# OpenResearchInstitute/ka9q-sdr

Measured on AMD Instinct MI355X. Metric: input Msamples/s + channels @ real-time, 16384-pt overlap-save, higher is better.
Workload: dtype f32

## Files before the change

ka9q_sdr_amd/csrc/kq_bank.cpp:

```cpp
#include <cstdarg>

#include "kq_bank.hpp"

using namespace kq::bank;

namespace {
thread_local std::string g_err;

int ilog2(unsigned v) {
  int l = 0;
  while ((1u << l) < v) l++;
  return l;
}
}

void kq_internal_set_error(const char *fmt, ...) {
  char buf[512];
  va_list ap;
  va_start(ap, fmt);
  vsnprintf(buf, sizeof buf, fmt, ap);
  va_end(ap);
  g_err = buf;
}

// ... 255 lines not shown
    if (b->alloc(&b->pl2[k].filt, C * B * g.olen, true)) return -1;
    if (b->alloc(&b->pl2[k].n0raw, C * B, true)) return -1;
    if (b->alloc(&b->pl2[k].if_power, B * (1 + kq::kEnergySplitMax), true)) return -1;
    if (g.pl_n > 0 && b->alloc(&b->pl2[k].plout, C * B * g.pl_l, true)) return -1;
  }
  b->pl = b->pl2[0];
  if (b->alloc(&b->energy_state, 2, true)) return -1;
  if (kq::full16k_paired_supported(g) && b->alloc(&b->win_paired, (size_t)(g.M - 1) + (size_t)B * g.L, true)) return -1;
  for (int *&l : b->list_dev)
    if (b->alloc(&l, C, true)) return -1;
  for (kq_bank::CtlQueue &q : b->ctl)
    for (int k = 0; k < kq_bank::CtlQueue::kDepth; k++)
      if (b->alloc_pinned(&q.buf[k], kq_bank::CtlQueue::kBytes) || b->new_event(&q.applied[k], hipEventDisableTiming)) return -1;
  {
    kq_bank::DesignQueue &d = b->dq;
    size_t const per_job = (size_t)g.Ndec * sizeof(float2);
    d.max_jobs = (unsigned)std::max<size_t>(1, std::min<size_t>(kq_bank::DesignQueue::kMax, ((size_t)64 << 20) / per_job));
    if (b->alloc(&d.scratch, (size_t)d.max_jobs * g.Ndec, true)) return -1;
    if (b->alloc(&d.ng_next, 2 * C, true)) return -1;
    for (int k = 0; k < kq_bank::DesignQueue::kDepth; k++)
      if (b->alloc_pinned(&d.pin[k], kq_bank::DesignQueue::kMax * (sizeof(kq::DesignJob) + sizeof(kq::DesignTarget))) ||
          b->new_event(&d.read[k], hipEventDisableTiming))
        return -1;
    for (hipEvent_t &e : d.ng_moved)
      if (b->new_event(&e, hipEventDisableTiming)) return -1;
    if (g.Ndec <= 16384 && kq::design_prepare(g.olen, g.Mdec)) return -1;
  }
  if (b->alloc(&b->list_active_dev, C, true)) return -1;
  if (b->alloc(&b->list_active_ds_dev, C, true)) return -1;
  if (b->alloc(&b->chd.fflags, C, true)) return -1;
  if (b->alloc(&b->list_unswept_dev, C, true)) return -1;
  if (b->alloc(&b->list_swept_dev, C, true)) return -1;
  if (b->fwd_mode == KQ_FWD_PRUNED && b->alloc(&b->chan_tw, C * kq::pruned_table_elems(g), true)) return -1;
  KQ_TRY(hipStreamSynchronize(b->stream));
  if (g.pl_n > 0) {
    int const PL_M = g.pl_n - g.pl_l + 1;
    std::vector<kq::cfloat> r(g.pl_n / 2 + 1, kq::cfloat(0, 0));
    for (int j = 0; j <= g.pl_n / 2; j++) {
      float const f = (float)j * g.dsamprate / g.Ndec;
      if (f > 0 && f < 300) r[j] = 1;
    }
    if (kq::window_rfilter(g.pl_l, PL_M, r, 2.0)) return -1;
    KQ_TRY(hipMemcpy(b->chd.plresp, r.data(), r.size() * sizeof(float2), hipMemcpyHostToDevice));
  }
  {
    std::vector<float> nanv(C, NAN);
    KQ_TRY(hipMemcpy(b->chd.plfreq, nanv.data(), C * sizeof(float), hipMemcpyHostToDevice));
  }
  return 0;
}
}

kq_bank *kq_bank_create(const kq_bank_config *cfg) {
  if (create_check(cfg)) return nullptr;
  kq::DeviceScope dev_scope_(cfg->device);
  {
    int cur = -1;
    if (hipGetDevice(&cur) != hipSuccess || cur != cfg->device) {
      kq_internal_set_error("hipSetDevice(%d) failed", cfg->device);
      return nullptr;
    }
  }
  kq_bank *b = new kq_bank();
  b->cfg = *cfg;
  b->chans.reserve(cfg->max_channels);
  if (create_geometry(b) || create_alloc(b)) {
// ... 79 lines not shown
```

ka9q_sdr_amd/csrc/kq_bank.hpp:

```cpp
#pragma once
#include <hip/hip_runtime.h>

#include <chrono>
#include <cmath>
#include <cstdio>
#include <cstdlib>
#include <cstring>
#include <map>
#include <mutex>
#include <string>
#include <unordered_map>
#include <vector>

#include "kq_design.hpp"
#include "kq_device.hpp"
#include "kq_host.hpp"

#define LAUNCH_CHECK(what)                                                                        \
  do {                                                                                            \
    hipError_t e_ = hipGetLastError();                                                            \
    if (e_ != hipSuccess) {                                                                       \
      kq_internal_set_error("kernel launch failed in %s: %s", what, hipGetErrorString(e_));       \
      return -1;                                                                                  \
    }                                                                                             \
// ... 55 lines not shown
  int histx_dev[kq::kOldLevels] = {-1, -1, -1, -1};
  static_assert(kq::kOldLevels == 4, "histx_dev's initialiser");
  bool active = true;
  kq_out_rtp_state out_rtp{};
  int out_type;
  std::vector<kq::cfloat> resp, aresp;
  float noise_gain;
  int pll_slot = -1;
  int n0slot = -1;
  int lk = -1, lpos = -1, apos = -1;
  bool patched = false;
  double r_eff = 0;
};

struct EventPair {
  hipEvent_t a, b;
};

}

struct kq_bank : kq::HostSide {
  std::recursive_mutex mu;
  kq_bank_config cfg;
  kq::Geom g;
  int fwd_mode = KQ_FWD_FULL;
  uint64_t calls = 0;
  int64_t n_abs = 0;
  int64_t out_abs = 0;
  unsigned last_blocks = 0;

  const float2 *tw = nullptr;
  float2 *chan_tw = nullptr;
  bool chan_tw_dirty = true;
  kq::ChanDev chd{};
  kq::Planes pl{};
  float *energy_state = nullptr;
  float2 *win_paired = nullptr;
  bool use64k = false;
  kq::Big64 big{};
  float *fmout = nullptr;
  float *fm_hist[2] = {nullptr, nullptr};
  int fm_hist_cur = 0;

  int timing = 0;
  kq_host_timing host_acc = {};
  const char *worst_holder = "";
  std::vector<kq::bank::EventPair> ev_filter, ev_demod, ev_ingest;
  size_t ev_used[3] = {0, 0, 0};
  kq_timing acc = {};

  struct CtlQueue {
    static constexpr size_t kBytes = 1u << 20, kMaxRec = 4096;
    static constexpr int kDepth = 4;
    unsigned char *buf[kDepth] = {};
    hipEvent_t applied[kDepth] = {};
    bool applied_set[kDepth] = {};
    int cur = 0;
    unsigned nrec = 0;
    size_t used = 0;
    std::unordered_map<unsigned long long, unsigned> at;
  };
  CtlQueue ctl[2];
  struct DesignQueue {
    static constexpr unsigned kMax = 1024;
    static constexpr int kDepth = 4;
    unsigned char *pin[kDepth] = {};
// ... 228 lines not shown
```

ka9q_sdr_amd/csrc/kq_bank_call.cpp:

```cpp
#include "kq_bank.hpp"

using namespace kq::bank;

namespace kq::bank {

void harvest_slot(kq_bank *b, int slot) {
  if (!b->stage_timed[slot]) return;
  b->stage_timed[slot] = false;
  float ms = 0;
  if (hipEventElapsedTime(&ms, b->stage_t0[slot], b->stage_ev[slot]) == hipSuccess && ms > 0) {
    b->acc.filter_ms += ms;
    if (ms > b->acc.filter_max_ms) {
      b->acc.filter_max_ms = ms;
      b->acc.filter_max_submit_ms = b->stage_submit_ms[slot];
      b->acc.filter_max_launch = b->stage_launch[slot];
    }
  } else
    (void)hipGetLastError();
}

void note_retune(kq_bank *b, int ch) {
  HostChan &h = b->chans[ch];
  int64_t const hist = (int64_t)b->g.M - 1;
  if (h.retuned && h.hist_old == hist) return;
// ... 327 lines not shown
    for (int c = 0; c < k.C; c++) {
      if (!b->chans[c].active) continue;
      bool const isb = b->chans[c].cfg.demod_type == KQ_LINEAR_DEMOD && b->chans[c].cfg.isb;
      for (unsigned i = 0; i < k.nblocks; i++) {
        const float2 *X = k.spectrum + (size_t)i * g.N;
        size_t const cb = (size_t)c * g.max_blocks + i;
        if (b->cfg.compute_n0)
          kq::launch_n0_single(b->stream, X, g.N, g.samprate, b->chans[c].cfg.low, b->chans[c].cfg.high, k.pl.n0raw + cb);
        kq::launch_slave_bank(b->stream, X, k.chd.resp + (size_t)c * g.Ndec, k.pl.filt + cb * g.olen, g.N, g.Ndec, g.olen, isb ? 2 : 1,
                              b->tw, g.tw_log2);
      }
    }
  } else if (b->fwd_mode == KQ_FWD_PRUNED) {
    if (b->chan_tw_dirty) {
      kq::launch_pruned_tables(b->stream, g, k.chd, b->chan_tw, k.C);
      b->chan_tw_dirty = false;
    }
    if (kq::pruned_carries_iir(g)) iir_arm(b, k);
    kq::launch_filter_pruned(b->stream, g, k.chd, k.pl, k.window, b->chan_tw, act.n, nblocks, k.swept_pruned, act.list, b->big.iir);
    b->big.iir = kq::IirArgs{};
    if (k.nret > 0) {
      if (g.N > 16384)
        kq::launch_filter_split(b->stream, g, k.chd, k.pl, k.window, b->tw, k.nret, (int)k.nredo, k.retune_list);
      else
        full_launch(b, k, k.nret, (int)k.nredo, k.retune_list, 0, false);
    }
  } else if (b->use64k) {
    launch64k(b, k, act.n, nblocks, act.list, k.plain);
    if (k.plain && k.nret > 0) launch64k(b, k, k.nret, (int)k.nredo, k.retune_list, false);
  } else if (g.N > 16384) {
    kq::launch_filter_split(b->stream, g, k.chd, k.pl, k.window, b->tw, k.C, nblocks, nullptr);
  } else {
    int const steady_variant = k.swept_steady ? 2 : k.plain ? 1 : 0;
    if (k.mixed) {
      full_launch(b, k, (int)b->list_unswept_host.size(), nblocks, b->list_unswept_dev, 1);
      full_launch(b, k, (int)b->list_swept_host.size(), nblocks, b->list_swept_dev, steady_variant);
    } else {
      full_launch(b, k, act.n, nblocks, act.list, steady_variant);
    }
    if (k.use16k && (k.plain || k.mixed || k.swept_steady) && k.nret > 0)
      full_launch(b, k, k.nret, (int)k.nredo, k.retune_list, 0);
  }
}

int launch_energy_and_filter(kq_bank *b, Call &k) {
  kq::Geom const &g = b->g;
  int const slot = k.slot, pp = k.pp;
  if (ctl_flush(b, CTL_FILTER, b->stream)) return -1;
  {
    Scope t(b, 2, b->stream);
    kq::launch_block_energy_sum(b->stream, k.spectrum ? nullptr : k.window + (g.M - 1), g.L, k.spectrum ? 0 : (int)k.nblocks,
                                k.pl.if_power + b->cfg.max_blocks,
                                b->stage_host[slot], b->osc_dev2[pp],
                                k.nret ? k.ret_off + k.nret * sizeof(int) : 8 * k.Cmax * sizeof(double) + k.nblocks,
                                k.spectrum ? nullptr : k.paired, (int)(g.M - 1), k.steady ? b->osc_dev2[pp ^ 1] : nullptr, (unsigned)k.C,
                                (unsigned)k.Cmax, (double)(k.n_w - b->planes_n_w), (double)(b->out_abs - b->planes_out_abs),
                                b->stage_host[slot] + b->patch_off, k.npatch, b->stage_host[slot] + b->bits_off);
  }
  LAUNCH_CHECK("IF power");
  if (b->timing) {
    KQ_TRY(hipEventRecord(b->stage_t0[slot], b->stream));
    b->stage_timed[slot] = true;
    b->stage_h0[slot] = std::chrono::steady_clock::now();
    b->stage_launch[slot] = b->acc.filter_launches;
  }
  static bool const iir_in_filter_off = getenv("KQ_IIR_IN_FILTER") && atoi(getenv("KQ_IIR_IN_FILTER")) == 0;
// ... 210 lines not shown
```

ka9q_sdr_amd/csrc/kq_bank_chan.cpp:

```cpp
#include "kq_bank.hpp"

using namespace kq::bank;

namespace {

int out_type_of(const kq_channel_config &k) { return (k.demod_type == KQ_LINEAR_DEMOD && k.isb) ? kq::FT_CROSS_CONJ : kq::FT_COMPLEX; }
bool is_pll(const kq_channel_config &c) { return c.demod_type == KQ_LINEAR_DEMOD && c.pll; }

int pll_admit(kq_bank *b, const kq_channel_config &m) {
  float const samptime = (float)b->g.D / (float)b->g.samprate;
  float const binsize = (float)(1. / (65536 * samptime));
  int const nbins = 2 * (int)round((m.square ? 2 : 1) * 300.f / binsize) + 1;
  if (nbins > 4096) {
    kq_internal_set_error("output rate too low for the PLL search window (%d bins > 4096)", nbins);
    return -1;
  }
  return 0;
}

int pll_acquire(kq_bank *b, int c) {
  size_t const Cmax = b->cfg.max_channels;
  if (!b->list_pll_dev) {
    if (alloc_cleared(b, &b->list_pll_dev, Cmax) || alloc_cleared(b, &b->pll_slot_dev, Cmax) ||
        alloc_cleared(b, &b->pll_chunks_dev, (size_t)kq_bank::kMaxPllChunks))
// ... 72 lines not shown
  int c = (int)b->chans.size();
  for (int k = 0; k < (int)b->chans.size(); k++)
    if (!b->chans[k].active) {
      c = k;
      break;
    }
  if ((size_t)c >= b->cfg.max_channels) {
    kq_internal_set_error("bank is full (%u channels)", b->cfg.max_channels);
    return -1;
  }
  if (check_channel_config(b, *cfg)) return -1;
  if (is_pll(*cfg) && pll_admit(b, *cfg)) return -1;
  HostChan h;
  h.cfg = *cfg;
  h.out_type = out_type_of(*cfg);
  set_oscillators(b, h, *cfg);
  bool const appended = c == (int)b->chans.size();
  if (appended)
    b->chans.push_back(h);
  else
    b->chans[c] = h;
  if ((is_pll(*cfg) && pll_acquire(b, c)) || upload_channel(b, c) || queue_design(b, c)) {
    pll_release(b, c);
    release_n0slot(b, b->chans[c].n0slot);
    b->chans[c].n0slot = -1;
    if (appended)
      b->chans.pop_back();
    else
      b->chans[c].active = false;
    return -1;
  }
  if (lists_add(b, c)) return -1;
  b->chan_tw_dirty = true;
  b->chans[c].r_eff = 0;
  b->n_active++;
  b->cache_any = true;
  b->sweep_lists_dirty = true;
  note_patch(b, c);
  return c;
}

int kq_bank_add_channels(kq_bank *b, const kq_channel_config *cfgs, unsigned n, int *indices) {
  BankScope dev_scope_(b);
  if (!b || (!cfgs && n)) {
    kq_internal_set_error("NULL argument");
    return -1;
  }
  if (n == 0) return 0;
  bool holes = false, any_pll = false, any_nan = false;
  for (HostChan const &h : b->chans) holes = holes || !h.active;
  for (unsigned i = 0; i < n; i++) any_pll = any_pll || is_pll(cfgs[i]);
  for (unsigned i = 0; i < n; i++) any_nan = any_nan || std::isnan(cfgs[i].kaiser_beta);
  if (holes || any_pll || any_nan || n < 4) {
    std::vector<int> got;
    for (unsigned i = 0; i < n; i++) {
      int const c = kq_bank_add_channel(b, &cfgs[i]);
      if (c < 0) {
        std::string const why = kq_last_error();
        for (size_t k = got.size(); k-- > 0;) (void)kq_bank_remove_channel(b, got[k]);
        kq_internal_set_error("%s", why.c_str());
        return -1;
      }
      got.push_back(c);
      if (indices) indices[i] = c;
    }
    return (int)n;
// ... 124 lines not shown
    int const nsub = b->use64k ? 4 : 1;
    std::vector<int> slots(n);
    unsigned taken = 0;
    auto fill = [&]() -> int {
      for (unsigned i = 0; i < n; i++) {
        bool fresh = false;
        int const slot = acquire_n0slot(b, cfgs[i].low, cfgs[i].high, &fresh);
        hs[i].n0slot = slots[i] = slot;
        if (slot < 0) return -1;
        taken = i + 1;
        if (fresh) {
          std::vector<unsigned long long> m;
          std::vector<unsigned> meta;
          build_n0mask(b, cfgs[i].low, cfgs[i].high, m, meta);
          KQ_TRY(hipMemcpy(b->chd.n0lane + (size_t)slot * nsub * 256, m.data(), m.size() * sizeof(m[0]), hipMemcpyHostToDevice));
          KQ_TRY(hipMemcpy(b->chd.n0meta + (size_t)slot * nsub, meta.data(), meta.size() * sizeof(unsigned), hipMemcpyHostToDevice));
        }
      }
      KQ_TRY(hipMemcpy(b->chd.n0slot + c0, slots.data(), n * sizeof(int), hipMemcpyHostToDevice));
      return 0;
    };
    if (fill()) {
      for (unsigned i = 0; i < taken; i++) release_n0slot(b, slots[i]);
      return -1;
    }
  }
  for (unsigned i = 0; i < n; i++) {
    b->chans.push_back(std::move(hs[i]));
    if (indices) indices[i] = (int)(c0 + i);
  }
  b->lists_dirty = true;
  b->osc_dirty = true;
  b->chan_tw_dirty = true;
  return (int)n;
}

int kq_bank_remove_channel(kq_bank *b, int ch) {
  BankScope dev_scope_(b);
  if (!valid_ch(b, ch)) {
    kq_internal_set_error("bad channel");
    return -1;
  }
  HostChan &h = b->chans[ch];
  pll_release(b, ch);
  if (lists_remove(b, ch)) return -1;
  h.active = false;
  h.retuned = false;
  h.hist_old = 0;
  for (int64_t &n : h.hist_oldx) n = 0;
  h.patched = false;
  release_n0slot(b, h.n0slot);
  h.n0slot = -1;
  b->n_active--;
  b->n_swept -= h.r_eff != 0;
  b->n_fast -= std::fabs(h.r_eff) > sweep_limit(b);
  b->cache_any = b->n_active > 0;
  b->sweep_lists_dirty = true;
  h.r_eff = 0;
  h.lo2 = h.dop = h.shift = h.lo2_old = h.dop_old = Osc{};
  for (int l = 0; l < kq::kOldLevels; l++) h.lo2_oldx[l] = h.dop_oldx[l] = Osc{};
  h.out_rtp = kq_out_rtp_state{};
  while (!b->chans.empty() && !b->chans.back().active) b->chans.pop_back();
  return 0;
}

int kq_bank_channel_active(const kq_bank *b, int ch) {
// ... 55 lines not shown
}

int kq_bank_set_linear_options(kq_bank *b, int ch, int isb, int channels) {
  BankScope dev_scope_(b);
  if (!valid_ch(b, ch) || (channels != 1 && channels != 2)) {
    kq_internal_set_error("bad channel, or channels not 1 or 2");
    return -1;
  }
  HostChan &h = b->chans[ch];
  if (h.cfg.demod_type != KQ_LINEAR_DEMOD) {
    kq_internal_set_error("not a linear channel");
    return -1;
  }
  if ((h.cfg.isb != 0) == (isb != 0) && h.cfg.channels == channels) return 0;
  h.cfg.isb = isb != 0;
  h.cfg.channels = channels;
  h.out_type = out_type_of(h.cfg);
  int const flags = channel_flags(h.cfg);
  if (ctl_put(b, CTL_FILTER, b->chd.fflags + ch, &flags, sizeof(int))) return -1;
  if (ctl_put(b, CTL_DEMOD, b->chd.flags + ch, &flags, sizeof(int))) return -1;
  return 0;
}

int kq_bank_set_second_lo(kq_bank *b, int ch, double hz) {
  BankScope dev_scope_(b);
  if (!valid_ch(b, ch) || std::isnan(hz)) {
    kq_internal_set_error("bad channel or NaN");
    return -1;
  }
  note_retune(b, ch);
  b->chans[ch].cfg.second_lo = hz;
  b->chans[ch].lo2.set(hz == 0 ? 0.0 : hz / b->g.samprate, 0.0, b->n_abs);
  b->chan_tw_dirty = true;
  note_patch(b, ch);
  return 0;
}

int kq_bank_set_doppler(kq_bank *b, int ch, double hz, double hz_per_s) {
  BankScope dev_scope_(b);
  if (!valid_ch(b, ch) || std::isnan(hz) || std::isnan(hz_per_s)) {
    kq_internal_set_error("bad channel or NaN");
    return -1;
  }
  double const fs = b->g.samprate;
  note_retune(b, ch);
  b->chans[ch].cfg.doppler = hz;
  b->chans[ch].cfg.doppler_rate = hz_per_s;
  b->chans[ch].dop.set(-hz / fs, -hz_per_s / (fs * fs), b->n_abs);
  b->chan_tw_dirty = true;
  note_patch(b, ch);
  return 0;
}

int kq_bank_set_shift(kq_bank *b, int ch, double hz) {
  BankScope dev_scope_(b);
  if (!valid_ch(b, ch) || std::isnan(hz)) {
    kq_internal_set_error("bad channel or NaN");
    return -1;
  }
  b->chans[ch].cfg.shift = hz;
  b->chans[ch].shift.set(hz == 0 ? 0.0 : hz * b->g.D / (double)b->g.samprate, 0.0, b->out_abs);
  note_patch(b, ch);
  return 0;
}

int kq_bank_set_n0(kq_bank *b, int ch, float n0) {
  BankScope dev_scope_(b);
  if (!valid_ch(b, ch)) {
    kq_internal_set_error("bad channel");
    return -1;
  }
  if (ctl_put(b, CTL_DEMOD, b->chd.n0 + ch, &n0, sizeof n0)) return -1;
  return 0;
}

int kq_bank_set_filter(kq_bank *b, int ch, float low, float high, float beta) {
  BankScope dev_scope_(b);
  if (!valid_ch(b, ch)) {
    kq_internal_set_error("bad channel");
    return -1;
  }
  if (std::isnan(low) || std::isnan(high)) {
// ... 17 lines not shown
```

ka9q_sdr_amd/csrc/kq_device.hpp:

```cpp
#pragma once
#include "kq_energy.hpp"
#include <hip/hip_runtime.h>
#include <stdint.h>

#include <functional>

#include "../../include/ka9q_hip.h"

struct filter_in;

namespace kq {

enum { FLAG_FLAT = 1, FLAG_ISB = 2, FLAG_STEREO = 4, FLAG_SQUARE = 8 };

struct PllState {
  double c_phase, c_freq;
  double f_phase, f_freq;
  float integrator, delta_f, snr, foffset, cphase;
  int lock_count, pll_lock, fft_samples, fft_ptr;
};

struct FftDim {
  int n;
  int log2n;
// ... 16 lines not shown
  float2 *side;
};

struct Geom {
  int N, L, M, D;
  FftDim dN, dNdec, dPl;
  int Ndec, olen, Mdec;
  int log2N, log2Ndec;
  int samprate;
  int tw_log2;
  int max_blocks;
  float dsamprate;
  int pl_n, pl_l;
};

constexpr int kOldLevels = 4;

struct ChanDev {
  int *mode;
  int *flags;
  int *fflags;
  float *low, *high;
  float2 *resp;
  float2 *aresp;
  float *fm_gain;
  float *headroom;
  float *recovery;
  int *hangmax;
  float *noise_gain;
  unsigned long long *n0lane;
  unsigned *n0meta;
  int *n0slot;
  double *lo_phase, *lo_freq, *lo_rate;
  double *hist_phase, *hist_freq, *hist_rate;
  int *hist_len;
  int *hist2_len;
  double *hist2_osc;
  double *sh_phase, *sh_freq;
  float2 *fm_state;
  float *lastaudio;
  int *sq_count;
  float *ahist;
  float *foffset, *pdev;
  float *gain;
  int *hang;
  float *dc;
  float *n0;
  float2 *plresp;
  float *plring;
  int *pl_ptr, *pl_last;
  float *plfreq;
};

struct Planes {
  float2 *filt;
  float *audio;
  kq_chan_status *status;
  float *n0raw;
  float *if_power;
  float *plout;
};

struct DeviceScope {
  int prev = -1;
  bool switched = false;
  explicit DeviceScope(int device) {
// ... 17 lines not shown
void launch_ingest(hipStream_t s, const void *src, int format, float2 *dst, size_t nsamples, float scale);
constexpr int kEnergySplitMax = 16;
int block_energy_split(int L);
void launch_block_energy_sum(hipStream_t s, const float2 *newsamples, int L, int nblocks, float *sums, const void *params_host,
                             void *params_dev, size_t params_bytes, float2 *paired, int hist, const double *prev_planes = nullptr,
                             unsigned nchan = 0, unsigned cmax = 0, double adv = 0, double adv_out = 0, const void *patch_records_host = nullptr,
                             int npatch = 0, const void *patch_bits_host = nullptr);
void launch_ctl_apply(hipStream_t s, const void *queue_host, int nrec);
void launch_block_energy_iir(hipStream_t s, const float *sums, int L, int nblocks, const unsigned char *update, float *energy_state,
                             float *if_power);
void launch_pcm(hipStream_t s, const Geom &g, const Planes &pl, short *pcm, unsigned *mask, int nchan, int nblocks,
                const int *chan_list);
void launch_filter_full(hipStream_t s, const Geom &g, const ChanDev &ch, const Planes &pl, const float2 *window,
                        const float2 *tw, int nchan, int nblocks, int compute_n0, float2 *spec_dump, int spec_ch,
                        const int *chan_list);
bool split_supported(const Geom &g);
void launch_filter_split(hipStream_t s, const Geom &g, const ChanDev &ch, const Planes &pl, const float2 *window,
                         const float2 *tw, int nchan, int nblocks, const int *chan_list);
struct Big64 {
  unsigned long long *sync;
  float2 *n0part;
  float2 *xs;
  int *err;
  unsigned epoch;
  IirArgs iir;
};
bool full16k_supported(const Geom &g);
constexpr int kFull16kHalf = 16;
constexpr int full16k_bin(int t) { return (t >> 5) + 32 * (t & 31); }
void launch_filter_full16k(hipStream_t s, const Geom &g, const ChanDev &ch, const Planes &pl, const float2 *window,
                           const float2 *tw, int nchan, int nblocks, int compute_n0, float2 *spec_dump, int spec_ch,
                           const int *chan_list, int plain, const float2 *window_paired, const Big64 &big);
bool full16k_paired_supported(const Geom &g);
bool full64k_supported(const Geom &g);
void launch_filter_full64k(hipStream_t s, const Geom &g, const ChanDev &ch, const Planes &pl, const float2 *window,
                           const float2 *tw, int nchan, int nblocks, int compute_n0, float2 *spec_dump, int spec_ch,
                           const int *chan_list, bool plain, bool swept, const float2 *window_paired, const Big64 &big);
double full16k_sweep_limit();
double full64k_sweep_limit();
bool pruned_supported(const Geom &g);
void launch_filter_pruned(hipStream_t s, const Geom &g, const ChanDev &ch, const Planes &pl, const float2 *window,
                          const float2 *chan_tw, int nchan, int nblocks, bool swept, const int *chan_list, const IirArgs &iir = IirArgs{});
bool pruned_carries_iir(const Geom &g);
void launch_pruned_tables(hipStream_t s, const Geom &g, const ChanDev &ch, float2 *chan_tw, int nchan);
size_t pruned_table_elems(const Geom &g);
size_t demod_fm_lds_bytes(const Geom &g);
void launch_demod_fm(hipStream_t s, const Geom &g, const ChanDev &ch, const Planes &pl, const float2 *tw, const int *list_fm,
                     int n_fm, int nblocks, int compute_n0, float *fmout, const float *fm_hist_in, float *fm_hist_out);
void launch_pl_track(hipStream_t s, const Geom &g, const ChanDev &ch, const Planes &pl, const float2 *tw, const int *list_fm,
                     int n_fm, int nblocks);
bool demod64_supported(const Geom &g);
void launch_demod64(hipStream_t s, const Geom &g, const ChanDev &ch, const Planes &pl, const int *list_fm, int n_fm,
                    const int *list_am, int n_am, const int *list_lin, int n_lin, int nblocks, int compute_n0);
void launch_demod_pll(hipStream_t s, const Geom &g, const ChanDev &ch, const Planes &pl, const float2 *tw, const int *list_pll,
                      int n_pll, const PllChunk *chunks, const int *slot_of, int nblocks, int compute_n0);
void launch_fft_single(hipStream_t s, const float2 *in, float2 *out, const FftDim &d, int sign, const float2 *tw, int tw_log2);
int launch_fft_large(hipStream_t s, const float2 *in, float2 *out, float2 *tmp, int N, int sign, const float2 *tw, int tw_log2);
void launch_n0_single(hipStream_t s, const float2 *fdomain, int N, int samprate, float low, float high, float *out);
void launch_slave_single(hipStream_t s, const float2 *fdomain, const float2 *resp, float2 *out, int N, int Ndec,
                         int in_real, int out_type, const float2 *tw, int tw_log2);
void launch_slave_bank(hipStream_t s, const float2 *fdomain, const float2 *resp, float2 *out, int N, int Ndec, int olen,
                       int out_type, const float2 *tw, int tw_log2);


int compat_snapshot_window(struct filter_in *master, float2 *dst, unsigned *block);
int compat_snapshot_spectrum(struct filter_in *master, float2 *dst, unsigned *block);
// ... 4 lines not shown
```

ka9q_sdr_amd/csrc/kq_full16k.hip:

```cpp
#include "kq_device.hpp"
#include "kq_ldsfft.hpp"
#include <cmath>
#include <type_traits>

#include "kq_lane.hpp"
#include "kq_regfft.hpp"

#ifdef KQ_TIMELINE
__device__ unsigned long long kq_timeline[64][8][12];
#define KQ_STAMP(i)                                                                        \
  do {                                                                                     \
    __builtin_amdgcn_sched_barrier(0);                                                     \
    if (blockIdx.y == (gridDim.y > 40 ? 40 : gridDim.y / 2) && (blockIdx.x & 15) == 0 && (blockIdx.x >> 4) < 64 &&      \
        (threadIdx.x & 63) == 0)                                                           \
      kq_timeline[blockIdx.x >> 4][threadIdx.x >> 6][i] = clock64();                       \
    __builtin_amdgcn_sched_barrier(0);                                                     \
  } while (0)
extern "C" int kq_debug_timeline(unsigned long long *dst) {
  return hipMemcpyFromSymbol(dst, HIP_SYMBOL(kq_timeline), sizeof(kq_timeline)) == hipSuccess ? 0 : -1;
}
#else
#define KQ_STAMP(i)
#endif

// ... 27 lines not shown
  v4f const q = __builtin_bit_cast(v4f, __builtin_amdgcn_raw_buffer_load_b128(r, (int)lane_off, (int)row_off, 0));
  a = (v2f){q.x, q.y};
  b = (v2f){q.z, q.w};
}

constexpr int kTabP1 = 0;
constexpr int kTabEpi = kTabP1 + 10 * kT;
constexpr int kTabTw2 = kTabEpi + 5 * 64, kTabSize = kTabTw2 + 512;
constexpr int kTw2Pitch = 34;

__device__ __forceinline__ void twiddle32(v2f (&v)[32], const v2f (&tlo)[3], const v2f (&thi)[7], v2f c) {
  v2f lo[4];
  lo[0] = c;
#pragma unroll
  for (int l = 1; l < 4; l++) lo[l] = pk_cmul(c, tlo[l - 1]);
#pragma unroll
  for (int l = 0; l < 4; l++) v[l] = pk_cmul(v[l], lo[l]);
#pragma unroll
  for (int h = 1; h < 8; h++) {
#pragma unroll
    for (int l = 0; l < 4; l++) v[4 * h + l] = pk_cmul(v[4 * h + l], pk_cmul(thi[h - 1], lo[l]));
  }
}
__device__ __forceinline__ void twiddle32_fetch(v2f (&tlo)[3], v2f (&thi)[7], rsrc_t tab, int t) {
  v2f e[10];
#pragma unroll
  for (int j = 0; j < 5; j++) buf_ld4(e[2 * j], e[2 * j + 1], tab, (unsigned)t * 16u, (unsigned)(kTabP1 + 2 * kT * j) * 8u);
#pragma unroll
  for (int l = 0; l < 3; l++) tlo[l] = e[l];
#pragma unroll
  for (int h = 0; h < 7; h++) thi[h] = e[3 + h];
}

__device__ __forceinline__ v2f phasor2(double turns) {
  float2 const p = phasor_turns(turns);
  return (v2f){p.x, p.y};
}

constexpr double kSweepLimit64k = 1.1e-11;
constexpr double kSweepLimit16k = 4.8e-11;

__device__ __forceinline__ void sibling_exchange(unsigned long long *slots, int r4, unsigned value, unsigned tag, float *out,
                                                 int *err) {
  int const t = threadIdx.x;
  if (t == 0)
    __hip_atomic_store(slots + r4, ((unsigned long long)tag << 32) | value, __ATOMIC_RELAXED, __HIP_MEMORY_SCOPE_AGENT);
  if (t < 4) {
    unsigned long long w = 0;
    int it = 0;
    for (;;) {
      w = __hip_atomic_load(slots + t, __ATOMIC_RELAXED, __HIP_MEMORY_SCOPE_AGENT);
      if ((unsigned)(w >> 32) == tag || ++it > (1 << 18)) break;
      __builtin_amdgcn_s_sleep(8);
    }
    if ((unsigned)(w >> 32) != tag) {
      *err = 1;
      w = 0x7fc00000u;
    }
    out[t] = __uint_as_float((unsigned)w);
  }
  __syncthreads();
}

}

template <bool N0, bool DUMP, int PLAIN, bool PAIRED, int BIG, int EPI>
__global__ __launch_bounds__(kT, 4) void k_filter_full16k(Geom g, ChanDev ch, Planes pl, const float2 *__restrict__ window,
                                                       const float2 *__restrict__ tw, const float2 *__restrict__ tab,
                                                       float2 *__restrict__ spec_dump, int spec_ch,
                                                       const int *__restrict__ chan_list, Big64 big) {
  extern __shared__ __attribute__((aligned(16))) float2 xch[];
  __shared__ __attribute__((aligned(16))) float2 stab[(kT / 64) * (BIG ? 128 : 32)];
  __shared__ float sib_f[BIG ? 12 : 1];
  constexpr int kNfull = BIG ? 4 * kN : kN;
  int const r4 = BIG ? (int)(blockIdx.x & 3) : 0;
  __shared__ __attribute__((aligned(16))) float2 tw2[16 * kTw2Pitch];
  __shared__ float red_f[2][kT / 64];
  __shared__ float red_c[kT / 64];
  __shared__ int red_i[2][kT / 64];
  int const t = threadIdx.x;
  int const Ndec = g.Ndec;
  KQ_STAMP(0);
  __builtin_amdgcn_s_setprio(3);
  v2f v[32];
  rsrc_t const xr = make_rsrc(window + (size_t)blockIdx.y * g.L, kNfull * (unsigned)sizeof(float2));
  unsigned const toff = (unsigned)t * (unsigned)sizeof(float2);
  auto load_rows = [&](int first, int last) {
    if constexpr (PAIRED) {
#pragma unroll
      for (int n1 = first; n1 < last; n1 += 2)
        buf_ld4(v[rfft::bitrev5(n1)], v[rfft::bitrev5(n1 + 1)], xr, 2 * toff, (unsigned)(n1 / 2) * (unsigned)(1024 * sizeof(float2)));
    } else {
#pragma unroll
      for (int n1 = first; n1 < last; n1++) v[rfft::bitrev5(n1)] = buf_ld2(xr, toff, (unsigned)n1 * (unsigned)(512 * sizeof(float2)));
    }
  };
  auto load_window = [&]() { load_rows(0, 32); };
  rsrc_t const tabr = make_rsrc(tab, kTabSize * (unsigned)sizeof(float2));
  v2f tlo[3], thi[7];
  int const cidx = BIG ? (int)(blockIdx.x >> 2) : (int)blockIdx.x;
  int const c = chan_list ? chan_list[cidx] : cidx, b = blockIdx.y;
  v2f pt = (v2f){1.f, 0.f};
  if constexpr (BIG != 0) {
    double const ph0 = ch.lo_phase[c], f0 = ch.lo_freq[c], rs = ch.lo_rate[c];
    double const hp0 = ch.hist_phase[c], hf0 = ch.hist_freq[c], hr = ch.hist_rate[c];
// ... 66 lines not shown
            v2f const Uu = n1 ? rfft::pk_fma(S, (v2f){n1 / 32.f, n1 / 32.f}, W) : W;
            asm("v_pk_fma_f32 %0, %1, %2, %3 op_sel:[1,0,0] op_sel_hi:[0,1,1] neg_lo:[0,1,0]" : "=v"(z) : "v"(Uu), "v"(kb), "v"(S));
          } else {
            z = pk_cmul(x[0], w[0]);
            z = rfft::pk_cmadd(x[1], w[1], z);
            z = rfft::pk_cmadd(x[2], w[2], z);
            z = rfft::pk_cmadd(x[3], w[3], z);
          }
          v[rfft::bitrev5(n1)] = z;
        }
        if (i + 2 < 16) issue(i + 2, slot);
      }
    } else {
      OlderOsc older;
      load_older(ch, c, b * g.L, n_old > 0, older);
#pragma unroll
      for (int n1 = 0; n1 < 32; n1++) {
        v2f acc = (v2f){0.f, 0.f};
        for (int j = 0; j < 4; j++) {
          int const i = 16384 * j + 512 * n1 + t;
          double const m = mbase + i;
          bool const old = i < n_old;
          double pp = old ? hp0 : ph0, ff = old ? hf0 : f0, rr = old ? hr : rs;
          pick_older(older, i, pp, ff, rr);
          double turns = pp + ff * m;
          if (rr != 0.0) turns += rr * (0.5 * m * (m - 1.0));
          turns -= (double)(r4 * (512 * n1 + t)) * (1.0 / 65536.0) + 0.25 * (double)(r4 * j);
          acc = rfft::pk_cmadd(buf_ld2(xr, toff, (unsigned)(32 * j + n1) * (unsigned)(512 * sizeof(float2))), phasor2(turns), acc);
        }
        v[rfft::bitrev5(n1)] = acc;
      }
    }
  }
  if constexpr (PLAIN && BIG == 0) {
    double const ph0 = ch.lo_phase[c], f0 = ch.lo_freq[c];
    double const rs = PLAIN == 2 ? ch.lo_rate[c] : 0.0;
    load_rows(0, 12);
    __builtin_amdgcn_sched_barrier(0);
    float2 *const sw = stab + (t >> 6) * 32;
    if ((t & 63) < 32) {
      double const R = (double)(512 * (t & 63));
      double turns = f0 * R;
      if constexpr (PLAIN == 2) turns += rs * (0.5 * R * (R - 1.0) + R * ((double)b * g.L + (double)(t & ~63)));
      sw[t & 63] = phasor_turns(turns);
    }
    __builtin_amdgcn_sched_barrier(0);
    load_rows(12, 22);
    __builtin_amdgcn_sched_barrier(0);
    {
      double const A = (double)b * g.L + t;
      double turns = ph0 + f0 * A;
      if constexpr (PLAIN == 2) turns += rs * (0.5 * A * (A - 1.0));
      pt = phasor2(turns);
    }
    __builtin_amdgcn_sched_barrier(0);
    load_rows(22, 32);
  }
  twiddle32_fetch(tlo, thi, tabr, t);
  v2f const tw2_mine = buf_ld2(tabr, toff, (unsigned)kTabTw2 * 8u);
  KQ_STAMP(10);

  if constexpr (BIG == 0) {
    double const ph0 = ch.lo_phase[c], f0 = ch.lo_freq[c], r = ch.lo_rate[c];
    double const hp0 = ch.hist_phase[c], hf0 = ch.hist_freq[c], hr = ch.hist_rate[c];
    double const mbase = (double)b * g.L;
    int const n_old = (hp0 != ph0 || hf0 != f0 || hr != r) ? ch.hist_len[c] - b * g.L : 0;
    bool const retuned = n_old > 0;
    if (PLAIN || (r == 0.0 && !retuned)) {
      float2 *const sw = stab + (t >> 6) * 32;
      if constexpr (!PLAIN) {
        load_window();
        if ((t & 63) < 32) sw[t & 63] = phasor_turns(f0 * (double)(512 * (t & 63)));
        pt = phasor2(ph0 + f0 * (mbase + t));
      }
      KQ_STAMP(11);
      __builtin_amdgcn_fence(__ATOMIC_RELEASE, "wavefront");
      __builtin_amdgcn_wave_barrier();
      __builtin_amdgcn_fence(__ATOMIC_ACQUIRE, "wavefront");
      if constexpr (PLAIN == 2) {
        float const kbf = (float)(2.0 * M_PI * 512.0 * r * (double)(t & 63));
        v2f const kb = (v2f){kbf, kbf};
        v2f th = (v2f){0.f, 0.f};
#pragma unroll
        for (int n1 = 1; n1 < 32; n1++) {
          v2f const y = pk_cmul(v[rfft::bitrev5(n1)], ld2(sw + n1));
          th = th + kb;
          v2f z;
          asm("v_pk_fma_f32 %0, %1, %2, %3 op_sel:[1,0,0] op_sel_hi:[0,1,1] neg_lo:[0,1,0]" : "=v"(z) : "v"(y), "v"(th), "v"(y));
          v[rfft::bitrev5(n1)] = z;
        }
      } else {
#pragma unroll
        for (int n1 = 1; n1 < 32; n1++) v[rfft::bitrev5(n1)] = pk_cmul(v[rfft::bitrev5(n1)], ld2(sw + n1));
      }
    } else if constexpr (!PLAIN) {
      OlderOsc older;
      load_older(ch, c, b * g.L, n_old > 0, older);
#pragma unroll
      for (int n1 = 0; n1 < 32; n1++) {
        int const i = 512 * n1 + t;
        double const m = mbase + i;
        bool const old = i < n_old;
        double pp = old ? hp0 : ph0, ff = old ? hf0 : f0, rr = old ? hr : r;
        pick_older(older, i, pp, ff, rr);
        double turns = pp + ff * m;
        if (rr != 0.0) turns += rr * (0.5 * m * (m - 1.0));
        v[rfft::bitrev5(n1)] = pk_cmul(buf_ld2(xr, toff, (unsigned)n1 * (unsigned)(512 * sizeof(float2))), phasor2(turns));
      }
    }
  }

  KQ_STAMP(1);
// ... 410 lines not shown
                              const int *__restrict__ chan_list, int compute_n0) {
  extern __shared__ __attribute__((aligned(16))) float2 G[];
  int const t = threadIdx.x, Ndec = g.Ndec;
  int const c = chan_list ? chan_list[blockIdx.x] : (int)blockIdx.x, b = blockIdx.y;
  size_t const cb = (size_t)c * g.max_blocks + b;
  if (compute_n0 && t == 0) {
    const float2 *p = big.n0part + cb * 4;
    float const tf = (p[0].x + p[1].x) + (p[2].x + p[3].x), bins = (p[0].y + p[1].y) + (p[2].y + p[3].y);
    float const avg = tf / bins;
    pl.n0raw[cb] = (float)(avg / (2.0 * 65536.0 * g.samprate));
  }
  const float2 *Xs = big.xs + cb * Ndec;
  const float2 *H = ch.resp + (size_t)c * Ndec;
  bool const isb = (ch.fflags[c] & FLAG_ISB) != 0;
  for (int p = t; p <= Ndec / 2; p += blockDim.x) {
    float2 gp = cmul(H[p], Xs[p]);
    if (p > 0 && p < Ndec / 2) {
      int const k = Ndec - p;
      float2 gn = cmul(H[k], Xs[k]);
      if (isb) {
        float2 const pos = gp, neg = gn;
        gp = cadd(pos, cconj(neg));
        gn = csub(neg, cconj(pos));
      }
      G[bitrev((unsigned)k, g.log2Ndec)] = gn;
    }
    G[bitrev((unsigned)p, g.log2Ndec)] = gp;
  }
  lds_fft<+1>(G, g.log2Ndec, tw, g.tw_log2);
  float2 *o = pl.filt + cb * g.olen;
  for (int i = t; i < g.olen; i += blockDim.x) o[i] = G[Ndec - g.olen + i];
}

bool full16k_supported(const Geom &g) {
  return g.N == kN && 2 * g.Ndec <= kXchElems && g.Ndec >= 4;
}

static const float2 *twiddle_tables() {
  return (const float2 *)upload_once(TABLE_FULL16K, kN, kTabSize * sizeof(float2), [](void *bytes) {
    float2 *h = (float2 *)bytes;
    auto w = [](long long e) {
      double const ang = -2.0 * M_PI * (double)(e % kN) / kN;
      return make_float2((float)cos(ang), (float)sin(ang));
    };
    for (int t = 0; t < kT; t++)
      for (int e = 0; e < 10; e++)
        h[kTabP1 + 2 * (kT * (e >> 1) + t) + (e & 1)] = e < 3 ? w((long long)(e + 1) * t) : w(4LL * (e - 2) * t);
    for (int n3 = 0; n3 < 16; n3++)
      for (int k2 = 0; k2 < 32; k2++) h[kTabTw2 + 32 * n3 + k2] = w(32LL * n3 * k2);
    for (int st = 1; st <= 5; st++)
      for (int t = 0; t < 64; t++) {
        int const half = 1 << st;
        double const ang = M_PI * (double)(t & (half - 1)) / half;
        h[kTabEpi + (st - 1) * 64 + t] = (t & half) ? make_float2((float)cos(ang), (float)sin(ang)) : make_float2(1.f, 0.f);
      }
  });
}

bool full16k_paired_supported(const Geom &g) {
  return (full16k_supported(g) || full64k_supported(g)) && g.L % 1024 == 0 && (g.M - 1) % 1024 == 0;
}

bool full64k_supported(const Geom &g) { return g.N == 4 * kN && g.Ndec >= 4 && g.Ndec <= 16384; }
double full64k_sweep_limit() { return kSweepLimit64k; }
double full16k_sweep_limit() { return kSweepLimit16k; }

void launch_filter_full16k(hipStream_t s, const Geom &g, const ChanDev &ch, const Planes &pl, const float2 *window,
                           const float2 *tw, int nchan, int nblocks, int compute_n0, float2 *spec_dump, int spec_ch,
                           const int *chan_list, int plain, const float2 *window_paired, const Big64 &big) {
  size_t const lds_bytes = (size_t)kXchElems * sizeof(float2);
  const float2 *tab = twiddle_tables();
  if (!tab) {
    launch_filter_full(s, g, ch, pl, window, tw, nchan, nblocks, compute_n0, spec_dump, spec_ch, chan_list);
    if (big.iir.sums)
      launch_block_energy_iir(s, big.iir.sums, big.iir.L, big.iir.nblocks, big.iir.update, big.iir.state, big.iir.if_power);
    return;
  }
  bool const n0 = compute_n0 && ch.n0lane && ch.n0meta;
  bool const dump = spec_dump != nullptr;
  bool const paired = plain && window_paired != nullptr;
  auto go = [&](auto kernel) {
    ensure_dynamic_lds((const void *)kernel, lds_bytes);
    hipLaunchKernelGGL(kernel, dim3(nchan, nblocks), dim3(kT), lds_bytes, s, g, ch, pl, paired ? window_paired : window, tw, tab,
                       spec_dump, spec_ch, chan_list, big);
  };
  int const epi = dump ? 0 : g.Ndec == 64 ? 1 : (g.Ndec >= 128 && g.Ndec <= 512) ? 2 : 0;
  auto pick3 = [&](auto n0c, auto dumpc, auto epic) {
    constexpr bool kN0 = decltype(n0c)::value, kDump = decltype(dumpc)::value;
    constexpr int kEpi = decltype(epic)::value;
    if (plain == 2)
      paired ? go(k_filter_full16k<kN0, kDump, 2, true, 0, kEpi>) : go(k_filter_full16k<kN0, kDump, 2, false, 0, kEpi>);
    else if (paired)
      go(k_filter_full16k<kN0, kDump, 1, true, 0, kEpi>);
    else
      plain ? go(k_filter_full16k<kN0, kDump, 1, false, 0, kEpi>) : go(k_filter_full16k<kN0, kDump, 0, false, 0, kEpi>);
  };
  auto pick = [&](auto n0c, auto dumpc) {
    if constexpr (decltype(dumpc)::value) {
      pick3(n0c, dumpc, std::integral_constant<int, 0>{});
    } else {
      if (epi == 1)
        pick3(n0c, dumpc, std::integral_constant<int, 1>{});
      else if (epi == 2)
        pick3(n0c, dumpc, std::integral_constant<int, 2>{});
      else
        pick3(n0c, dumpc, std::integral_constant<int, 0>{});
    }
  };
  using T = std::true_type;
  using F = std::false_type;
  if (n0)
    dump ? pick(T{}, T{}) : pick(T{}, F{});
// ... 45 lines not shown
```

Baseline: 383,000.

## Precompute per-channel row phasors in a small table for plain 16k filter

Adds a per-channel 32-entry row phasor table, filled by a small kernel when tuning changes (dirty flag) or on non-steady calls. The plain 16k filter kernel loads these through scalar constant-address loads into registers and multiplies with an SGPR-operand packed complex multiply. This replaces the per-block double-precision phasor computation, the LDS staging and the wave barrier. It costs an extra tiny launch on retune and 32 more registers per thread, which may reduce occupancy.

```diff
diff --git a/ka9q_sdr_amd/csrc/kq_bank.cpp b/ka9q_sdr_amd/csrc/kq_bank.cpp
--- a/ka9q_sdr_amd/csrc/kq_bank.cpp
+++ b/ka9q_sdr_amd/csrc/kq_bank.cpp
@@ -311,6 +311,7 @@
   if (b->alloc(&b->list_unswept_dev, C, true)) return -1;
   if (b->alloc(&b->list_swept_dev, C, true)) return -1;
   if (b->fwd_mode == KQ_FWD_PRUNED && b->alloc(&b->chan_tw, C * kq::pruned_table_elems(g), true)) return -1;
+  if (b->fwd_mode != KQ_FWD_PRUNED && kq::full16k_supported(g) && b->alloc(&b->chd.row_ph, C * 32, true)) return -1;
   KQ_TRY(hipStreamSynchronize(b->stream));
   if (g.pl_n > 0) {
     int const PL_M = g.pl_n - g.pl_l + 1;
diff --git a/ka9q_sdr_amd/csrc/kq_bank.hpp b/ka9q_sdr_amd/csrc/kq_bank.hpp
--- a/ka9q_sdr_amd/csrc/kq_bank.hpp
+++ b/ka9q_sdr_amd/csrc/kq_bank.hpp
@@ -111,6 +111,7 @@
   const float2 *tw = nullptr;
   float2 *chan_tw = nullptr;
   bool chan_tw_dirty = true;
+  bool row_ph_dirty = true;
   kq::ChanDev chd{};
   kq::Planes pl{};
   float *energy_state = nullptr;
diff --git a/ka9q_sdr_amd/csrc/kq_bank_call.cpp b/ka9q_sdr_amd/csrc/kq_bank_call.cpp
--- a/ka9q_sdr_amd/csrc/kq_bank_call.cpp
+++ b/ka9q_sdr_amd/csrc/kq_bank_call.cpp
@@ -383,6 +383,10 @@
     kq::launch_filter_split(b->stream, g, k.chd, k.pl, k.window, b->tw, k.C, nblocks, nullptr);
   } else {
     int const steady_variant = k.swept_steady ? 2 : k.plain ? 1 : 0;
+    if (k.use16k && (k.plain || k.mixed) && (b->row_ph_dirty || !k.steady)) {
+      kq::launch_full16k_rows(b->stream, k.chd, k.C);
+      b->row_ph_dirty = false;
+    }
     if (k.mixed) {
       full_launch(b, k, (int)b->list_unswept_host.size(), nblocks, b->list_unswept_dev, 1);
       full_launch(b, k, (int)b->list_swept_host.size(), nblocks, b->list_swept_dev, steady_variant);
diff --git a/ka9q_sdr_amd/csrc/kq_bank_chan.cpp b/ka9q_sdr_amd/csrc/kq_bank_chan.cpp
--- a/ka9q_sdr_amd/csrc/kq_bank_chan.cpp
+++ b/ka9q_sdr_amd/csrc/kq_bank_chan.cpp
@@ -128,6 +128,7 @@
   }
   if (lists_add(b, c)) return -1;
   b->chan_tw_dirty = true;
+  b->row_ph_dirty = true;
   b->chans[c].r_eff = 0;
   b->n_active++;
   b->cache_any = true;
@@ -318,6 +319,7 @@
   b->lists_dirty = true;
   b->osc_dirty = true;
   b->chan_tw_dirty = true;
+  b->row_ph_dirty = true;
   return (int)n;
 }
 
@@ -439,6 +441,7 @@
   b->chans[ch].cfg.second_lo = hz;
   b->chans[ch].lo2.set(hz == 0 ? 0.0 : hz / b->g.samprate, 0.0, b->n_abs);
   b->chan_tw_dirty = true;
+  b->row_ph_dirty = true;
   note_patch(b, ch);
   return 0;
 }
@@ -455,6 +458,7 @@
   b->chans[ch].cfg.doppler_rate = hz_per_s;
   b->chans[ch].dop.set(-hz / fs, -hz_per_s / (fs * fs), b->n_abs);
   b->chan_tw_dirty = true;
+  b->row_ph_dirty = true;
   note_patch(b, ch);
   return 0;
 }
diff --git a/ka9q_sdr_amd/csrc/kq_device.hpp b/ka9q_sdr_amd/csrc/kq_device.hpp
--- a/ka9q_sdr_amd/csrc/kq_device.hpp
+++ b/ka9q_sdr_amd/csrc/kq_device.hpp
@@ -72,6 +72,7 @@
   unsigned *n0meta;
   int *n0slot;
   double *lo_phase, *lo_freq, *lo_rate;
+  float2 *row_ph;
   double *hist_phase, *hist_freq, *hist_rate;
   int *hist_len;
   int *hist2_len;
@@ -155,6 +156,7 @@
                            const float2 *tw, int nchan, int nblocks, int compute_n0, float2 *spec_dump, int spec_ch,
                            const int *chan_list, int plain, const float2 *window_paired, const Big64 &big);
 bool full16k_paired_supported(const Geom &g);
+void launch_full16k_rows(hipStream_t s, const ChanDev &ch, int nchan);
 bool full64k_supported(const Geom &g);
 void launch_filter_full64k(hipStream_t s, const Geom &g, const ChanDev &ch, const Planes &pl, const float2 *window,
                            const float2 *tw, int nchan, int nblocks, int compute_n0, float2 *spec_dump, int spec_ch,
diff --git a/ka9q_sdr_amd/csrc/kq_full16k.hip b/ka9q_sdr_amd/csrc/kq_full16k.hip
--- a/ka9q_sdr_amd/csrc/kq_full16k.hip
+++ b/ka9q_sdr_amd/csrc/kq_full16k.hip
@@ -83,10 +83,18 @@
   for (int h = 0; h < 7; h++) thi[h] = e[3 + h];
 }
 
+__device__ __forceinline__ v2f pk_cmul_s(v2f a, v2f b) {
+  v2f t, d;
+  asm("v_pk_mul_f32 %0, %1, %2 op_sel_hi:[0,1]" : "=v"(t) : "v"(a), "s"(b));
+  asm("v_pk_fma_f32 %0, %1, %2, %3 op_sel:[1,1,0] op_sel_hi:[1,0,1] neg_lo:[1,0,0]" : "=v"(d) : "v"(a), "s"(b), "v"(t));
+  return d;
+}
+
 __device__ __forceinline__ v2f phasor2(double turns) {
   float2 const p = phasor_turns(turns);
   return (v2f){p.x, p.y};
 }
+__device__ __forceinline__ float2 row_phasor(double f0, int n1) { return phasor_turns(f0 * (double)(512 * n1)); }
 
 constexpr double kSweepLimit64k = 1.1e-11;
 constexpr double kSweepLimit16k = 4.8e-11;
@@ -121,7 +129,8 @@
                                                        float2 *__restrict__ spec_dump, int spec_ch,
                                                        const int *__restrict__ chan_list, Big64 big) {
   extern __shared__ __attribute__((aligned(16))) float2 xch[];
-  __shared__ __attribute__((aligned(16))) float2 stab[(kT / 64) * (BIG ? 128 : 32)];
+  constexpr bool kRowPlane = PLAIN == 1 && BIG == 0;
+  __shared__ __attribute__((aligned(16))) float2 stab[kRowPlane ? 1 : (kT / 64) * (BIG ? 128 : 32)];
   __shared__ float sib_f[BIG ? 12 : 1];
   constexpr int kNfull = BIG ? 4 * kN : kN;
   int const r4 = BIG ? (int)(blockIdx.x & 3) : 0;
@@ -254,17 +263,26 @@
       }
     }
   }
+  v2f srow[kRowPlane ? 32 : 1];
   if constexpr (PLAIN && BIG == 0) {
     double const ph0 = ch.lo_phase[c], f0 = ch.lo_freq[c];
     double const rs = PLAIN == 2 ? ch.lo_rate[c] : 0.0;
+    if constexpr (kRowPlane) {
+      typedef const float2 __attribute__((address_space(4))) *row_plane;
+      row_plane const rp = (row_plane)(ch.row_ph + (size_t)__builtin_amdgcn_readfirstlane(c) * 32);
+#pragma unroll
+      for (int n1 = 1; n1 < 32; n1++) srow[n1] = (v2f){rp[n1].x, rp[n1].y};
+    }
     load_rows(0, 12);
     __builtin_amdgcn_sched_barrier(0);
-    float2 *const sw = stab + (t >> 6) * 32;
-    if ((t & 63) < 32) {
-      double const R = (double)(512 * (t & 63));
-      double turns = f0 * R;
-      if constexpr (PLAIN == 2) turns += rs * (0.5 * R * (R - 1.0) + R * ((double)b * g.L + (double)(t & ~63)));
-      sw[t & 63] = phasor_turns(turns);
+    if constexpr (PLAIN == 2) {
+      float2 *const sw = stab + (t >> 6) * 32;
+      if ((t & 63) < 32) {
+        double const R = (double)(512 * (t & 63));
+        double turns = f0 * R;
+        turns += rs * (0.5 * R * (R - 1.0) + R * ((double)b * g.L + (double)(t & ~63)));
+        sw[t & 63] = phasor_turns(turns);
+      }
     }
     __builtin_amdgcn_sched_barrier(0);
     load_rows(12, 22);
@@ -289,17 +307,22 @@
     int const n_old = (hp0 != ph0 || hf0 != f0 || hr != r) ? ch.hist_len[c] - b * g.L : 0;
     bool const retuned = n_old > 0;
     if (PLAIN || (r == 0.0 && !retuned)) {
-      float2 *const sw = stab + (t >> 6) * 32;
+      float2 *const sw = stab + (kRowPlane ? 0 : (t >> 6) * 32);
       if constexpr (!PLAIN) {
         load_window();
-        if ((t & 63) < 32) sw[t & 63] = phasor_turns(f0 * (double)(512 * (t & 63)));
+        if ((t & 63) < 32) sw[t & 63] = row_phasor(f0, t & 63);
         pt = phasor2(ph0 + f0 * (mbase + t));
       }
       KQ_STAMP(11);
-      __builtin_amdgcn_fence(__ATOMIC_RELEASE, "wavefront");
-      __builtin_amdgcn_wave_barrier();
-      __builtin_amdgcn_fence(__ATOMIC_ACQUIRE, "wavefront");
-      if constexpr (PLAIN == 2) {
+      if constexpr (!kRowPlane) {
+        __builtin_amdgcn_fence(__ATOMIC_RELEASE, "wavefront");
+        __builtin_amdgcn_wave_barrier();
+        __builtin_amdgcn_fence(__ATOMIC_ACQUIRE, "wavefront");
+      }
+      if constexpr (kRowPlane) {
+#pragma unroll
+        for (int n1 = 1; n1 < 32; n1++) v[rfft::bitrev5(n1)] = pk_cmul_s(v[rfft::bitrev5(n1)], srow[n1]);
+      } else if constexpr (PLAIN == 2) {
         float const kbf = (float)(2.0 * M_PI * 512.0 * r * (double)(t & 63));
         v2f const kb = (v2f){kbf, kbf};
         v2f th = (v2f){0.f, 0.f};
@@ -776,6 +799,15 @@
   for (int i = t; i < g.olen; i += blockDim.x) o[i] = G[Ndec - g.olen + i];
 }
 
+__global__ void __launch_bounds__(256) k_full16k_rows(ChanDev ch, int nchan) {
+  int const i = (int)(blockIdx.x * blockDim.x + threadIdx.x);
+  if (i >= 32 * nchan) return;
+  ch.row_ph[i] = row_phasor(ch.lo_freq[i >> 5], i & 31);
+}
+void launch_full16k_rows(hipStream_t s, const ChanDev &ch, int nchan) {
+  if (nchan > 0 && ch.row_ph) hipLaunchKernelGGL(k_full16k_rows, dim3((32 * nchan + 255) / 256), dim3(256), 0, s, ch, nchan);
+}
+
 bool full16k_supported(const Geom &g) {
   return g.N == kN && 2 * g.Ndec <= kXchElems && g.Ndec >= 4;
 }
@@ -822,6 +854,7 @@
   }
   bool const n0 = compute_n0 && ch.n0lane && ch.n0meta;
   bool const dump = spec_dump != nullptr;
+  if (plain == 1 && !ch.row_ph) plain = 0;
   bool const paired = plain && window_paired != nullptr;
   auto go = [&](auto kernel) {
     ensure_dynamic_lds((const void *)kernel, lds_bytes);
```

After: 393,700, median of 6. 1.03x the previous value.
